# Jackie-Chou/MC-CNN-python

Measured on AMD Instinct MI355X. Metric: Mdisparities/s (HxWxD / s) end-to-end match.py timed region, images resident in HBM, higher is better.
Workload: dtype f32; 1 GPU; cfg2: 750x500 synthetic stereo pair, D=256, one pair per GPU; weights=converted reference checkpoint

## Files before the change

### include/mccnn.h

```cpp
#ifndef MCCNN_H
#define MCCNN_H

#include <stddef.h>
#include <stdint.h>

#ifdef __cplusplus
extern "C" {
#endif

typedef void *mccnn_stream_t;

#define MCCNN_ABI_VERSION 7

#define MCCNN_E_INVALID (-1)
#define MCCNN_E_UNSUPPORTED (-2)
#define MCCNN_E_SCRATCH (-3)

#define MCCNN_SIDE_LEFT 0
#define MCCNN_SIDE_RIGHT 1

int mccnn_version(void);
const char *mccnn_last_error_string(void);

#define MCCNN_CV_EXACT 0
#define MCCNN_CV_MFMA 1
int mccnn_cost_volume(const float *fl, const float *fr, int H, int W, int C, int D, float *lcv, float *rcv, int mode,
                      mccnn_stream_t stream);

int mccnn_cost_volume_hwd(const float *fl, const float *fr, int H, int W, int C, int D, float *lcv_hwd, float *rcv_hwd,
                          int mode, mccnn_stream_t stream);

size_t mccnn_decision_pack_bytes(int n_fc, int units, int mode);
int mccnn_decision_pack(const float *weights, int n_fc, int units, float weight_scale, int mode, void *packed,
                        mccnn_stream_t stream);
int mccnn_cost_volume_accurate(const float *aL, const float *aR, int H, int W, int C, int units, int n_fc, int D,
                               const void *packed, const float *biases, const float *w_final, float b_final,
                               float weight_scale, float *lcv, float *rcv, int mode, int *saturation_flag,
                               mccnn_stream_t stream);
int mccnn_cost_volume_accurate_hwd(const float *aL, const float *aR, int H, int W, int C, int units, int n_fc, int D,
                                   const void *packed, const float *biases, const float *w_final, float b_final,
                                   float weight_scale, float *lcv_hwd, float *rcv_hwd, int mode, int *saturation_flag,
                                   mccnn_stream_t stream);

int mccnn_cost_volume_fill(float *lcv, float *rcv, int D, int H, int W, int pixel_major, mccnn_stream_t stream);

typedef uint32_t mccnn_support_t;
size_t mccnn_support_bytes(int H, int W);
#define MCCNN_SUPPORT_UP(s) ((s) & 31u)
#define MCCNN_SUPPORT_DOWN(s) (((s) >> 5) & 31u)
#define MCCNN_SUPPORT_LEFT(s) (((s) >> 10) & 31u)
#define MCCNN_SUPPORT_RIGHT(s) (((s) >> 15) & 31u)
#define MCCNN_SUPPORT_COUNT(s) ((s) >> 20)
int mccnn_cross_arms(const float *image, int H, int W, float tau, int L, mccnn_support_t *support,
                     mccnn_stream_t stream);
int mccnn_cross_arms_pair(const float *image_left, const float *image_right, int H, int W, float tau, int L,
                          mccnn_support_t *support_left, mccnn_support_t *support_right, mccnn_stream_t stream);
int mccnn_cross_region_list(const mccnn_support_t *support, int H, int W, int L, int32_t *region,
                            mccnn_stream_t stream);

#define MCCNN_CBCA_SEPARABLE 0
#define MCCNN_CBCA_REFERENCE_ORDER 1
int mccnn_cbca_iter(const float *in, float *out, const mccnn_support_t *support, int D, int H, int W, int L, int order,
                    mccnn_stream_t stream);

int mccnn_cbca_iter_pair(const float *in_left, float *out_left, const mccnn_support_t *support_left,
                         const float *in_right, float *out_right, const mccnn_support_t *support_right, int D, int H,
                         int W, int L, int order, mccnn_stream_t stream);

int mccnn_cbca_iter_both(const float *in, float *out, const mccnn_support_t *support_self,
                         const mccnn_support_t *support_other, int D, int H, int W, int L, int side,
                         mccnn_stream_t stream);

int mccnn_cbca_iter_hwd(const float *in_hwd, float *out_hwd, const mccnn_support_t *support, int D, int H, int W, int L,
                        mccnn_stream_t stream);
int mccnn_cbca_iter_hwd_pair(const float *in_left, float *out_left, const mccnn_support_t *support_left,
                             const float *in_right, float *out_right, const mccnn_support_t *support_right, int D,
                             int H, int W, int L, mccnn_stream_t stream);

int mccnn_cbca_iter_hwd_pair_wta(const float *in_left, float *out_left, const mccnn_support_t *support_left,
                                 const float *in_right, float *out_right, const mccnn_support_t *support_right, int D,
                                 int H, int W, int L, float *disparity_left, float *disparity_right, int store_right,
                                 mccnn_stream_t stream);

// ... 116 lines not shown
```

### mc-cnn-python_amd/csrc/cost_volume.hip

```cpp
#include "common.h"

namespace mccnn {

constexpr int CV_TW = 64;
constexpr int CV_DT = 64;
constexpr int CV_C = 64;
#ifndef CVM_WAVES_PER_SIMD
#define CVM_WAVES_PER_SIMD 6
#endif
constexpr int CV_LD = 68;

template <bool PIXEL_MAJOR>
__global__ __launch_bounds__(256) void cost_volume_exact_kernel(const float *__restrict__ fl,
                                                                const float *__restrict__ fr, int H, int W, int D,
                                                                float *__restrict__ lcv, float *__restrict__ rcv, int Dp)
{
    __shared__ __attribute__((aligned(16))) float sR[(CV_TW + CV_DT - 1) * CV_LD];
    __shared__ __attribute__((aligned(16))) float sL[CV_TW * CV_LD];
    const int w0 = blockIdx.x * CV_TW, h = blockIdx.y, d0 = blockIdx.z * CV_DT;
    if (w0 + CV_TW - 1 < d0) return;
    const int tid = threadIdx.x;
    const size_t rowbase = (size_t)h * W;
    for (int i = tid; i < CV_TW * 16; i += 256) {
        const int px = i >> 4, c4 = i & 15;
// ... 506 lines not shown
    const bool left = blockIdx.y == 0;
    const int d = (int)blockIdx.z * 64 + lane;
    const int dmax = min((int)blockIdx.z * 64 + 63, D - 1);
    if ((int)blockIdx.z * 64 >= D) return;
    float *row = (left ? lcv : rcv) + (size_t)h * W * Dp;
    const __amdgpu_buffer_rsrc_t rs = __builtin_amdgcn_make_buffer_rsrc(row, 0, (int)((size_t)W * Dp * 4), 0x00020000);
    const unsigned pix = (unsigned)Dp * 4u;
    const int c_first = left ? dmax + 2 : max(W - dmax - 3, 0), nsteps = left ? c_first + 1 : W - c_first;
    auto col = [&](int t) { return left ? c_first - t : c_first + t; };
    const int voff = d < Dp ? d * 4 : kDrop;
    const int sto = d < D ? voff : kDrop;
    float x1 = 0.f, x2 = 0.f, x3 = 0.f;
    float buf[PF];
    const int dmin = (int)blockIdx.z * 64;
    const int nA = min(nsteps, left ? c_first - dmin + 1 : (W - dmin) - c_first);
    auto issue = [&](int slot, int t) {
        const int c = col(min(t, nA - 1));
        buf[slot] = __uint_as_float(__builtin_amdgcn_raw_buffer_load_b32(rs, voff, (unsigned)c * pix, 0));
    };
    auto third = [](float s) {
        const float zh = 0.3333333432674407958984375f;
        const float q = s * zh;
        const float r = __builtin_fmaf(-3.0f, q, s);
        const float q2 = __builtin_fmaf(r, zh, q);
        return (__builtin_fabsf(s) < __builtin_inff() && s != 0.f) ? q2 : s;
    };
    auto step = [&](int c, bool stored, float have) {
        float s = 0.f - x1;
        s = s - x2;
        s = s - x3;
        const float val = stored ? have : -third(s);
        if (left) { x3 = x2; x2 = x1; x1 = val; }
        else      { x1 = x2; x2 = x3; x3 = val; }
        __builtin_amdgcn_raw_buffer_store_b32(__float_as_uint(val), rs, stored ? kDrop : sto, (unsigned)c * pix, 0);
    };
    if (nA > 0) {
#pragma unroll
        for (int k = 0; k < PF; ++k) issue(k, k);
        for (int t0 = 0; t0 < nA; t0 += PF) {
#pragma unroll
            for (int k = 0; k < PF; ++k) {
                const int t = t0 + k;
                if (t < nA) {
                    const int c = col(t);
                    step(c, left ? c >= d : c < W - d, buf[k]);
                }
                issue(k, t + PF);
            }
        }
    }
    for (int t = max(nA, 0); t < nsteps; ++t) step(col(t), false, 0.f);
}

int launch_cost_volume_fill(float *lcv, float *rcv, int D, int H, int W, hipStream_t s, const char *what)
{
    if (D > 1)
        hipLaunchKernelGGL(cost_volume_fill_kernel, dim3(cdiv(H, 64), D - 1, 2), dim3(64), 0, s, lcv, rcv, D, H, W);
    return check_launch(what);
}

int launch_cost_volume_fill_hwd(float *lcv_hwd, float *rcv_hwd, int D, int Dp, int H, int W, hipStream_t s, const char *what)
{
    if (D > 1) {
#ifdef CV_FILL_FOUR_PER_LANE
        if (Dp <= 256)
            hipLaunchKernelGGL(cost_volume_fill_hwd_kernel<1>, dim3(H, 2), dim3(64), 0, s, lcv_hwd, rcv_hwd, D, Dp, H, W);
        else
            hipLaunchKernelGGL(cost_volume_fill_hwd_kernel<2>, dim3(H, 2), dim3(64), 0, s, lcv_hwd, rcv_hwd, D, Dp, H, W);
#else
        hipLaunchKernelGGL(cost_volume_fill_hwd_lanes_kernel, dim3(H, 2, cdiv(D, 64)), dim3(64), 0, s, lcv_hwd, rcv_hwd, D, Dp,
                           H, W);
#endif
    }
    return check_launch(what);
}

}

extern "C" int mccnn_cost_volume(const float *fl, const float *fr, int H, int W, int C, int D, float *lcv, float *rcv,
                                 int mode, mccnn_stream_t stream)
{
    using namespace mccnn;
    MCCNN_REQUIRE(fl && fr && lcv && rcv, MCCNN_E_INVALID, "mccnn_cost_volume: null pointer");
    MCCNN_REQUIRE(H > 0 && W > 0 && D > 0, MCCNN_E_INVALID, "mccnn_cost_volume: non-positive size");
    MCCNN_REQUIRE(C == CV_C, MCCNN_E_UNSUPPORTED, "mccnn_cost_volume: C=%d, kernels are built for 64 channels", C);
    MCCNN_REQUIRE(D <= W - 2, MCCNN_E_UNSUPPORTED,
                  "mccnn_cost_volume: D=%d needs W >= D+2 (the reference's border recurrence pf:106 is degenerate "
                  "beyond that), W=%d", D, W);
    hipStream_t s = (hipStream_t)stream;
    const dim3 block(256);
    if (mode == MCCNN_CV_EXACT) {
        const dim3 grid(cdiv(W, CV_TW), H, cdiv(D, CV_DT));
        hipLaunchKernelGGL(cost_volume_exact_kernel<false>, grid, block, 0, s, fl, fr, H, W, D, lcv, rcv, 0);
    } else if (mode == MCCNN_CV_MFMA) {
        const int nwt = cdiv(W, 64), nbands = cdiv(D + 63, 64) + 1;
        const long total = (long)nwt * nbands * H;
        MCCNN_REQUIRE(total <= 0x7fffffffL, MCCNN_E_UNSUPPORTED, "mccnn_cost_volume: %ld tiles exceed the grid", total);
        hipLaunchKernelGGL(cost_volume_mfma_kernel<false>, dim3((unsigned)total), block, 0, s, fl, fr, H, W, D, lcv, rcv, nwt,
                           nbands, (int)total, 0);
    } else {
        MCCNN_REQUIRE(false, MCCNN_E_INVALID, "mccnn_cost_volume: unknown mode %d", mode);
    }
    int rc = check_launch("mccnn_cost_volume");
    if (rc) return rc;
    return launch_cost_volume_fill(lcv, rcv, D, H, W, s, "mccnn_cost_volume(fill)");
}

extern "C" int mccnn_cost_volume_hwd(const float *fl, const float *fr, int H, int W, int C, int D, float *lcv_hwd,
                                     float *rcv_hwd, int mode, mccnn_stream_t stream)
{
    using namespace mccnn;
    MCCNN_REQUIRE(fl && fr && lcv_hwd && rcv_hwd, MCCNN_E_INVALID, "mccnn_cost_volume_hwd: null pointer");
    MCCNN_REQUIRE(H > 0 && W > 0 && D > 0, MCCNN_E_INVALID, "mccnn_cost_volume_hwd: non-positive size");
    MCCNN_REQUIRE(C == CV_C, MCCNN_E_UNSUPPORTED, "mccnn_cost_volume_hwd: C=%d, kernels are built for 64 channels", C);
    MCCNN_REQUIRE(D <= W - 2, MCCNN_E_UNSUPPORTED,
                  "mccnn_cost_volume_hwd: D=%d needs W >= D+2 (the reference's border recurrence pf:106 is degenerate "
                  "beyond that), W=%d", D, W);
    MCCNN_REQUIRE(mode == MCCNN_CV_EXACT || mode == MCCNN_CV_MFMA, MCCNN_E_INVALID, "mccnn_cost_volume_hwd: unknown mode %d",
                  mode);
#ifdef CV_FILL_FOUR_PER_LANE
    constexpr int kMaxD = 512;
#else
    constexpr int kMaxD = 1024;
#endif
    MCCNN_REQUIRE(D <= kMaxD, MCCNN_E_UNSUPPORTED, "mccnn_cost_volume_hwd: D=%d > %d", D, kMaxD);
    const int Dp = mccnn_hwd_pitch(D);
    MCCNN_REQUIRE((size_t)W * Dp * 4 < ((size_t)1 << 31), MCCNN_E_UNSUPPORTED,
                  "mccnn_cost_volume_hwd: a %d x %d row exceeds a buffer descriptor's reach", W, D);
    hipStream_t s = (hipStream_t)stream;
    if (mode == MCCNN_CV_MFMA) {
        const int nwt = cdiv(W, 64), nbands = cdiv(D + 63, 64) + 1;
        const long total = (long)nwt * nbands * H;
        MCCNN_REQUIRE(total <= 0x7fffffffL, MCCNN_E_UNSUPPORTED, "mccnn_cost_volume_hwd: %ld tiles exceed the grid", total);
        hipLaunchKernelGGL(cost_volume_mfma_kernel<true>, dim3((unsigned)total), dim3(256), 0, s, fl, fr, H, W, D, lcv_hwd,
                           rcv_hwd, nwt, nbands, (int)total, Dp);
    } else {
#ifdef CV_HWD_TILE_KERNEL
        const dim3 grid(cdiv(W, CV_TW), H, cdiv(D, CV_DT));
        hipLaunchKernelGGL(cost_volume_exact_kernel<true>, grid, dim3(256), 0, s, fl, fr, H, W, D, lcv_hwd, rcv_hwd, Dp);
#else
        const dim3 grid(cdiv(W, CVP_TW), H, 1);
        hipLaunchKernelGGL(cost_volume_exact_pairs_kernel, grid, dim3(256), 0, s, fl, fr, H, W, D, lcv_hwd, rcv_hwd, Dp);
#endif
    }
    int rc = check_launch("mccnn_cost_volume_hwd");
    if (rc) return rc;
    return launch_cost_volume_fill_hwd(lcv_hwd, rcv_hwd, D, Dp, H, W, s, "mccnn_cost_volume_hwd(fill)");
}

extern "C" int mccnn_cost_volume_fill(float *lcv, float *rcv, int D, int H, int W, int pixel_major, mccnn_stream_t stream)
{
    using namespace mccnn;
    MCCNN_REQUIRE(lcv && rcv, MCCNN_E_INVALID, "mccnn_cost_volume_fill: null pointer");
    MCCNN_REQUIRE(H > 0 && W > 0 && D > 0, MCCNN_E_INVALID, "mccnn_cost_volume_fill: non-positive size");
    MCCNN_REQUIRE(D <= W - 2, MCCNN_E_UNSUPPORTED, "mccnn_cost_volume_fill: D=%d needs W >= D+2, W=%d", D, W);
    if (!pixel_major) return launch_cost_volume_fill(lcv, rcv, D, H, W, (hipStream_t)stream, "mccnn_cost_volume_fill");
    const int Dp = mccnn_hwd_pitch(D);
    MCCNN_REQUIRE(D <= 1024, MCCNN_E_UNSUPPORTED, "mccnn_cost_volume_fill: D=%d > 1024", D);
    MCCNN_REQUIRE((size_t)W * Dp * 4 < ((size_t)1 << 31), MCCNN_E_UNSUPPORTED,
                  "mccnn_cost_volume_fill: a %d x %d row exceeds a buffer descriptor's reach", W, D);
    return launch_cost_volume_fill_hwd(lcv, rcv, D, Dp, H, W, (hipStream_t)stream, "mccnn_cost_volume_fill");
}
```

### mc-cnn-python_amd/src/_hipabi.py

```python
import ctypes
import os

import torch

_HERE = os.path.dirname(os.path.abspath(__file__))
LIB_PATH = os.environ.get("MCCNN_HIP_LIB") or os.path.join(os.path.dirname(_HERE), "lib", "libmccnn_hip.so")

MCCNN_ABI_VERSION = 7
MCCNN_CV_EXACT = 0
MCCNN_CV_MFMA = 1
MCCNN_CBCA_SEPARABLE = 0
MCCNN_CBCA_REFERENCE_ORDER = 1
MCCNN_SIDE_LEFT = 0
MCCNN_SIDE_RIGHT = 1
MCCNN_SGM_ACC_STORE = 0
MCCNN_SGM_ACC_ADD = 1
MCCNN_SGM_ACC_ADD_QUARTER = 2
MCCNN_E_INVALID = -1
MCCNN_E_UNSUPPORTED = -2
MCCNN_E_SCRATCH = -3

_vp = ctypes.c_void_p
_i = ctypes.c_int
_f = ctypes.c_float
_sz = ctypes.c_size_t

SIGNATURES = {
    "mccnn_version": (_i, []),
    "mccnn_last_error_string": (ctypes.c_char_p, []),
    "mccnn_cost_volume": (_i, [_vp, _vp, _i, _i, _i, _i, _vp, _vp, _i, _vp]),
    "mccnn_cost_volume_hwd": (_i, [_vp, _vp, _i, _i, _i, _i, _vp, _vp, _i, _vp]),
    "mccnn_cost_volume_fill": (_i, [_vp, _vp, _i, _i, _i, _i, _vp]),
    "mccnn_decision_pack_bytes": (_sz, [_i, _i, _i]),
    "mccnn_decision_pack": (_i, [_vp, _i, _i, _f, _i, _vp, _vp]),
    "mccnn_cost_volume_accurate": (_i, [_vp, _vp, _i, _i, _i, _i, _i, _i, _vp, _vp, _vp, _f, _f, _vp, _vp, _i, _vp, _vp]),
    "mccnn_cost_volume_accurate_hwd": (_i, [_vp, _vp, _i, _i, _i, _i, _i, _i, _vp, _vp, _vp, _f, _f, _vp, _vp, _i, _vp,
                                            _vp]),
    "mccnn_support_bytes": (_sz, [_i, _i]),
    "mccnn_cross_arms": (_i, [_vp, _i, _i, _f, _i, _vp, _vp]),
    "mccnn_cross_arms_pair": (_i, [_vp, _vp, _i, _i, _f, _i, _vp, _vp, _vp]),
    "mccnn_cross_region_list": (_i, [_vp, _i, _i, _i, _vp, _vp]),
    "mccnn_cbca_iter": (_i, [_vp, _vp, _vp, _i, _i, _i, _i, _i, _vp]),
    "mccnn_cbca_iter_pair": (_i, [_vp, _vp, _vp, _vp, _vp, _vp, _i, _i, _i, _i, _i, _vp]),
    "mccnn_cbca_iter_both": (_i, [_vp, _vp, _vp, _vp, _i, _i, _i, _i, _i, _vp]),
    "mccnn_cbca_iter_hwd": (_i, [_vp, _vp, _vp, _i, _i, _i, _i, _vp]),
    "mccnn_cbca_iter_hwd_pair": (_i, [_vp, _vp, _vp, _vp, _vp, _vp, _i, _i, _i, _i, _vp]),
    "mccnn_cbca_iter_hwd_pair_wta": (_i, [_vp, _vp, _vp, _vp, _vp, _vp, _i, _i, _i, _i, _vp, _vp, _i, _vp]),
    "mccnn_cbca_iter_hwd_long": (_i, [_vp, _vp, _vp, _i, _i, _i, _i, _vp]),
    "mccnn_cbca_iter_hwd_long_pair": (_i, [_vp, _vp, _vp, _vp, _vp, _vp, _i, _i, _i, _i, _vp]),
    "mccnn_cbca_prog_bytes": (_sz, [_i, _i, _i]),
    "mccnn_cbca_prog_build_pair": (_i, [_vp, _vp, _i, _i, _i, _i, _vp, _vp, _vp]),
    "mccnn_cbca_iter_prog_pair": (_i, [_vp, _vp, _vp, _vp, _vp, _vp, _vp, _vp, _i, _i, _i, _i, _vp]),
    "mccnn_cbca_prog_build_skip_pair": (_i, [_vp, _vp, _i, _i, _i, _i, _vp, _vp, _vp]),
    "mccnn_cbca_prog_build_both_pair": (_i, [_vp, _vp, _i, _i, _i, _i, _vp, _vp, _vp]),
    "mccnn_cbca_iter_prog_pair_skip": (_i, [_vp, _vp, _vp, _vp, _vp, _vp, _vp, _vp, _i, _i, _i, _i, _vp]),
    "mccnn_cbca_iter_prog": (_i, [_vp, _vp, _vp, _vp, _i, _i, _i, _i, _vp]),
    "mccnn_cbca_iter_prog_skip": (_i, [_vp, _vp, _vp, _vp, _i, _i, _i, _i, _vp]),
    "mccnn_cbca_iter_prog_refresh": (_i, [_vp, _vp, _vp, _vp, _i, _i, _i, _i, _vp]),
    "mccnn_cbca_iter_prog_pair_refresh": (_i, [_vp, _vp, _vp, _vp, _vp, _vp, _vp, _vp, _i, _i, _i, _i, _vp]),
    "mccnn_cbca_iter_prog_pair_wta": (_i, [_vp, _vp, _vp, _vp, _vp, _vp, _vp, _vp, _i, _i, _i, _i, _vp, _vp, _i, _vp]),
    "mccnn_wta_hwd": (_i, [_vp, _i, _i, _i, _vp, _vp]),
    "mccnn_subpixel_hwd": (_i, [_vp, _vp, _i, _i, _i, _i, _vp, _vp]),
    "mccnn_hwd_pitch": (_i, [_i]),
    "mccnn_dhw_to_hwd": (_i, [_vp, _vp, _i, _i, _i, _vp]),
    "mccnn_hwd_to_dhw": (_i, [_vp, _vp, _i, _i, _i, _vp]),
    "mccnn_sgm_scratch_bytes": (_sz, [_i, _i, _i]),
    "mccnn_sgm_pass": (_i, [_vp, _vp, ctypes.POINTER(_vp), ctypes.POINTER(_i), _i, _i, _i, _i, _i, _i,
                            _f, _f, _f, _f, _f, _vp, _sz, _vp]),
    "mccnn_sgm_flags": (_i, [_vp, _vp, _i, _i, _i, _i, _i, _f, _vp, _sz, _vp]),
    "mccnn_sgm_pass_flagged": (_i, [ctypes.POINTER(_vp), ctypes.POINTER(_i), _i, _i, _i, _i, _i, _i, _f, _f, _f, _f, _vp, _sz,
                                    _vp]),
    "mccnn_sgm_pass_accumulate": (_i, [ctypes.POINTER(_vp), ctypes.POINTER(_vp), ctypes.POINTER(_i), _i, _i, _i, _i, _i, _i,
                                       _f, _f, _f, _f, _i, _vp, _sz, _vp]),
    "mccnn_sgm_first_pass": (_i, [_vp, _vp, ctypes.POINTER(_vp), ctypes.POINTER(_vp), ctypes.POINTER(_i), _i, _i, _i,
                                  _i, _f, _f, _f, _f, _f, _vp, _sz, _vp]),
    "mccnn_wta": (_i, [_vp, _i, _i, _i, _vp, _vp]),
    "mccnn_lr_status": (_i, [_vp, _vp, _i, _i, _i, _vp, _vp]),
    "mccnn_interpolate": (_i, [_vp, _vp, _i, _i, _vp, _vp]),
    "mccnn_interpolate_ex": (_i, [_vp, _vp, _i, _i, _i, _i, _vp, _vp]),
    "mccnn_subpixel": (_i, [_vp, _vp, _i, _i, _i, _vp, _vp]),
    "mccnn_subpixel_ex": (_i, [_vp, _vp, _i, _i, _i, _i, _vp, _vp]),
    "mccnn_median": (_i, [_vp, _i, _i, _i, _i, _vp, _vp]),
    "mccnn_bilateral": (_i, [_vp, _vp, _i, _i, _i, _i, _vp, _f, _vp, _vp]),
    "mccnn_bias_act": (_i, [_vp, _vp, _i, _i, ctypes.c_long, _i, _vp]),
# ... 64 lines not shown
```

### mc-cnn-python_amd/src/stereo_device.py

```python
import ctypes
import math

import numpy as np
import torch

import _hipabi as hip


def _f32(x):
    return float(np.float32(x))


class StageTimer(object):

    def __init__(self, enabled=False):
        self.enabled = enabled
        self.records = []
        self.spans = []
        self._open = None

    def start(self, name):
        if not self.enabled:
            return
        ev = torch.cuda.Event(enable_timing=True)
# ... 79 lines not shown
    lib = hip.load()
    packed = torch.empty((lib.mccnn_conv3x3_split_weights_bytes(),), dtype=torch.uint8, device=w.device)
    hip.check(lib.mccnn_conv3x3_split_pack(hip.ptr(w), scale, hip.ptr(packed), hip.stream()), "mccnn_conv3x3_split_pack")
    return packed, scale


def conv1_split(images, weight, bias, pad, act_scale=SPLIT_ACT_SCALE, sat_flag=None):
    N, H, W = images.shape
    assert tuple(weight.shape) == (64, 1, 3, 3) and images.is_contiguous() and weight.is_contiguous()
    out = torch.empty((N, H + 2 * pad - 2, W + 2 * pad - 2, 256), dtype=torch.uint8, device=images.device)
    hip.check(hip.load().mccnn_conv1_split(hip.ptr(images), hip.ptr(weight), hip.ptr(bias), hip.ptr(out), N, H, W,
                                           int(pad), float(act_scale), hip.ptr(sat_flag) if sat_flag is not None else None,
                                           hip.stream()), "mccnn_conv1_split")
    return out


def conv3x3_split(x, packed, weight_scale, bias, last, act_scale=SPLIT_ACT_SCALE, sat_flag=None):
    N, Hi, Wi, rec = x.shape
    assert rec == 256 and x.dtype == torch.uint8 and x.is_contiguous()
    if last:
        out = torch.empty((N, Hi - 2, Wi - 2, 64), dtype=torch.float32, device=x.device)
    else:
        out = torch.empty((N, Hi - 2, Wi - 2, 256), dtype=torch.uint8, device=x.device)
    hip.check(hip.load().mccnn_conv3x3_split(hip.ptr(x), hip.ptr(packed), hip.ptr(bias), hip.ptr(out), N, Hi, Wi,
                                             float(weight_scale), float(act_scale), 1 if last else 0,
                                             hip.ptr(sat_flag) if sat_flag is not None else None, hip.stream()),
              "mccnn_conv3x3_split")
    return out


def cost_volume(fl, fr, ndisp, mode=hip.MCCNN_CV_EXACT, out=None):
    H, W, C = fl.shape
    if out is None:
        lcv = torch.empty((ndisp, H, W), dtype=torch.float32, device=fl.device)
        rcv = torch.empty((ndisp, H, W), dtype=torch.float32, device=fl.device)
    else:
        lcv, rcv = out
    hip.check(hip.load().mccnn_cost_volume(hip.ptr(fl), hip.ptr(fr), H, W, C, int(ndisp), hip.ptr(lcv), hip.ptr(rcv),
                                           int(mode), hip.stream()), "mccnn_cost_volume")
    return lcv, rcv


def cost_volume_hwd(fl, fr, ndisp, out=None, mode=hip.MCCNN_CV_EXACT):
    H, W, C = fl.shape
    dp = hwd_pitch(ndisp)
    if out is None:
        lcv = torch.zeros((H, W, dp), dtype=torch.float32, device=fl.device)
        rcv = torch.zeros((H, W, dp), dtype=torch.float32, device=fl.device)
    else:
        lcv, rcv = out
    hip.check(hip.load().mccnn_cost_volume_hwd(hip.ptr(fl), hip.ptr(fr), H, W, C, int(ndisp), hip.ptr(lcv), hip.ptr(rcv),
                                               int(mode), hip.stream()), "mccnn_cost_volume_hwd")
    return lcv, rcv


DECISION_UNITS = 384
DECISION_MAPS = (64, 112)
DECISION_FC_LAYERS = (3, 4)
DECISION_MAX_D = 1024
DECISION_LIBRARY_BYTES = 256 << 20


def decision_kernel_refusal(net, W, D):
    if net.num_conv_feature_maps not in DECISION_MAPS:
        return "%d feature maps (the decision kernel serves %s)" % (net.num_conv_feature_maps, " or ".join(
            str(c) for c in DECISION_MAPS))
    if net.num_fc_units != DECISION_UNITS:
        return "%d units per hidden layer (the decision kernel is built for %d)" % (net.num_fc_units, DECISION_UNITS)
    if net.num_fc_layers not in DECISION_FC_LAYERS:
        return "%d fully-connected layers (the decision kernel serves 3 or 4)" % net.num_fc_layers
    if D < 2 or D > DECISION_MAX_D:
        return "ndisp=%d outside [2, %d]" % (D, DECISION_MAX_D)
    if D > W - 2:
        return "ndisp=%d needs an image at least ndisp + 2 pixels wide (W=%d)" % (D, W)
    return None


def decision_pack(weights, n_fc, mode):
    lib = hip.load()
    w = weights.detach().contiguous().float()
    units = int(w.shape[-1])
    nbytes = int(lib.mccnn_decision_pack_bytes(int(n_fc), units, int(mode)))
    if nbytes == 0 or tuple(w.shape) != (n_fc - 1, units, units):
        raise hip.MccnnHipError("mccnn_decision_pack: %d fc layers of %d units are outside the decision kernel's "
                                "envelope (3 or 4 layers of %d units)" % (n_fc, units, DECISION_UNITS))
    m = float(w.abs().max())
    scale = 2.0 ** math.floor(math.log2(1024.0 / m)) if m > 0.0 and math.isfinite(m) else 1.0
    packed = torch.empty((nbytes,), dtype=torch.uint8, device=w.device)
    hip.check(lib.mccnn_decision_pack(hip.ptr(w), int(n_fc), units, scale, int(mode), hip.ptr(packed), hip.stream()),
              "mccnn_decision_pack")
    return packed, scale


def cost_volume_fill(lcv, rcv, ndisp, pixel_major):
    H, W = (lcv.shape[0], lcv.shape[1]) if pixel_major else (lcv.shape[1], lcv.shape[2])
    hip.check(hip.load().mccnn_cost_volume_fill(hip.ptr(lcv), hip.ptr(rcv), int(ndisp), H, W, 1 if pixel_major else 0,
                                                hip.stream()), "mccnn_cost_volume_fill")
    return lcv, rcv


def accurate_scores_library(net, aL, aR, ndisp, lcv, rcv, pixel_major, budget=DECISION_LIBRARY_BYTES):
    H, W, U = aL.shape
    ws = [w.detach() for w in net.fc_weights]
    bs = [b.detach() for b in net.fc_biases]
    lv = lcv.permute(2, 0, 1) if pixel_major else lcv
    rv = rcv.permute(2, 0, 1) if pixel_major else rcv
# ... 634 lines not shown


DEFAULT_HP = dict(cbca_intensity=0.02, cbca_distance=14, cbca_num_iterations1=2, cbca_num_iterations2=16,
                  sgm_P1=2.3, sgm_P2=55.9, sgm_Q1=4, sgm_Q2=8, sgm_D=0.08, sgm_V=1.5, blur_sigma=6,
                  blur_threshold=2)


SGM_MAX_D = 1024
COST_VOLUME_HWD_MAX_D = 1024
DECISION_AUTO = "kernel"


def check_envelope(H, W, D):
    H, W, D = int(H), int(W), int(D)
    if H < 1 or W < 1:
        raise ValueError("%dx%d: empty image" % (W, H))
    if D < 2 or D > SGM_MAX_D:
        raise ValueError("ndisp=%d outside [2, %d]: SGM is built for at most %d disparities" % (D, SGM_MAX_D, SGM_MAX_D))
    if D > W - 2:
        raise ValueError("ndisp=%d needs an image at least ndisp + 2 = %d pixels wide, got W=%d" % (D, D + 2, W))


def workspace_bytes(H, W, D, pixel_major=True, cbca_kernel="auto", pairs_in_flight=1, arch="fast",
                    fc_units=DECISION_UNITS):
    check_envelope(H, W, D)
    lib = hip.load()
    H, W, D = int(H), int(W), int(D)
    dp = (D + 3) & ~3
    n = 4 * H * W * dp * 4
    n += 5 * int(lib.mccnn_sgm_scratch_bytes(H, W, D))
    n += 2 * int(lib.mccnn_support_bytes(H, W))
    n += H * W * 4 + 6 * H * W * 4
    if pixel_major and cbca_kernel != "hwd":
        n += 2 * int(lib.mccnn_cbca_prog_bytes(D, H, W))
    if arch not in ("fast", "accurate"):
        raise ValueError("arch must be 'fast' or 'accurate'")
    if arch == "accurate":
        n += 2 * H * W * int(fc_units) * 4
    return n * max(1, int(pairs_in_flight))


def _require_device_memory(nbytes, what):
    free, _total = torch.cuda.mem_get_info()
    avail = free + torch.cuda.memory_reserved() - torch.cuda.memory_allocated()
    if nbytes > avail:
        raise RuntimeError("%s needs %.2f GB of device memory, %.2f GB are available" % (what, nbytes / 1e9, avail / 1e9))


class StereoMatcher(object):

    def __init__(self, net, hp=None, cv_mode=hip.MCCNN_CV_EXACT, cbca_order=hip.MCCNN_CBCA_REFERENCE_ORDER,
                 feature_tile_rows=None, extras=None, features="auto", layout="auto", cbca_kernel="auto",
                 on_saturation="fallback", skip_unit_regions=True, two_chains=True, free_chains=True, refresh_first=True,
                 sgm_flags_once=True, decision="auto"):
        self.device = hip.require_device()
        self.net = net
        self.hp = dict(DEFAULT_HP)
        if hp:
            self.hp.update(hp)
        self.cv_mode = cv_mode
        self.cbca_order = cbca_order
        self.feature_tile_rows = feature_tile_rows
        if features not in ("auto", "miopen", "split_f16"):
            raise ValueError("features must be 'auto', 'miopen' or 'split_f16'")
        if features == "split_f16" and feature_tile_rows is not None:
            raise ValueError("row banding is implemented for the library convolutions only")
        if features == "auto":
            features = "split_f16" if (feature_tile_rows is None and net.supports_split_features()) else "miopen"
        self.features = features
        if decision not in ("auto", "kernel", "library"):
            raise ValueError("decision must be 'auto', 'kernel' or 'library'")
        self.accurate = hasattr(net, "fc_weights")
        self.decision = decision
        if self.accurate and features == "split_f16":
            raise ValueError("the split-operand feature kernels are built for the fast network")
        if layout not in ("auto", "plane_major"):
            raise ValueError("layout must be 'auto' or 'plane_major'")
        self.layout = layout
        if cbca_kernel not in ("auto", "prog", "hwd"):
            raise ValueError("cbca_kernel must be 'auto', 'prog' or 'hwd'")
        self.cbca_kernel = cbca_kernel
        if on_saturation not in ("fallback", "raise", "ignore"):
            raise ValueError("on_saturation must be 'fallback', 'raise' or 'ignore'")
        self.on_saturation = on_saturation
        self._library_twin = None
        self._decision_ran = None
        self.skip_unit_regions = bool(skip_unit_regions)
        self.two_chains = bool(two_chains)
        self.free_chains = bool(free_chains)
        self.refresh_first = bool(refresh_first)
        self.sgm_flags_once = bool(sgm_flags_once)
        self.extras = dict(both_view_support=False, interpolation_directions=4, occlusion_from_left=False,
                           numpy1_promotion=False, sgm_independent_directions=False)
        if extras:
            unknown = set(extras) - set(self.extras)
            if unknown:
                raise ValueError("unknown extras: %s" % sorted(unknown))
            self.extras.update(extras)
        self._ws = {}
        self._graphs = {}
        self._side = None
        self._right = None
        self._ingest = None

    def _right_stream(self):
        if self._right is None:
            self._right = torch.cuda.Stream()
        return self._right

    def features_saturated(self, reset=True):
        return self.net.split_saturated(reset)

    def saturation_checked(self):
        return self.features == "split_f16" or (self.accurate and self._decision_ran == "kernel")

    def saturation_notice(self):
        if self.accurate:
            return "activations left the matrix-core decision kernel's range: {} repeated on the float32 library decision route"
        return ("activations left the matrix-core feature kernels' range: {} repeated with the float32 library "
                "convolutions")

    def workspace(self, H, W, D):
        key = (H, W, D)
        ws = self._ws.get(key)
        if ws is None:
            need = workspace_bytes(H, W, D, self.pixel_major(), self.workspace_cbca_kernel(H, W, D),
                                   arch="accurate" if self.accurate else "fast",
                                   fc_units=self.net.num_fc_units if self.accurate else DECISION_UNITS)
            self._ws, self._graphs = {}, {}
            _require_device_memory(need, "StereoMatcher: the workspace of a %dx%d pair with ndisp=%d" % (W, H, D))
            dp = hwd_pitch(D)
            n = H * W * dp
            dev = self.device
            ws = dict(
                vol=[torch.empty((n,), dtype=torch.float32, device=dev) for _ in range(4)],
                scratch=sgm_scratch(H, W, D, dev),
                sgm_flags=[sgm_scratch(H, W, D, dev) for _ in SGM_DIRECTIONS],
                sup_l=support_buffer(H, W, dev), sup_r=support_buffer(H, W, dev),
                status=torch.empty((H, W), dtype=torch.int32, device=dev),
                maps=torch.empty((6, H, W), dtype=torch.float32, device=dev),
            )
            if self.accurate:
                ws["halves"] = tuple(torch.empty((H, W, self.net.num_fc_units), dtype=torch.float32, device=dev)
                                     for _ in range(2))
# ... 42 lines not shown
            if redo is not None:
                return redo
        return res

    def _side_work(self, ws, L, R, D, want_flags):
        hp = self.hp
        if self._side is None:
            self._side = torch.cuda.Stream()
        self._side.wait_stream(torch.cuda.current_stream())
        with torch.cuda.stream(self._side):
            sup_l, sup_r = cross_arms_pair(L, R, hp["cbca_intensity"], hp["cbca_distance"], ws["sup_l"], ws["sup_r"])
            if ws["progs"] is not None:
                cbca_prog_build_pair(sup_l, sup_r, D, hp["cbca_distance"], ws["progs"],
                                     "both" if self.skip_unit_regions else "full")
            flag_planes = sgm_flag_planes(L, R, D, hp["sgm_D"], out=ws["sgm_flags"]) if want_flags else None
            ready = torch.cuda.Event()
            ready.record(self._side)
        return sup_l, sup_r, flag_planes, ready

    def _side_work_timed(self, ws, L, R, D, timer):
        hp = self.hp
        timer.start("cross_arms")
        sup_l, sup_r = cross_arms_pair(L, R, hp["cbca_intensity"], hp["cbca_distance"], ws["sup_l"], ws["sup_r"])
        timer.stop()
        if ws["progs"] is not None:
            timer.start("cbca_prog_build")
            cbca_prog_build_pair(sup_l, sup_r, D, hp["cbca_distance"], ws["progs"])
            timer.stop()
        return sup_l, sup_r

    def decision_route(self, W, D):
        if self.decision == "library":
            return "library"
        why = decision_kernel_refusal(self.net, W, D)
        if why is None:
            return DECISION_AUTO if self.decision == "auto" else "kernel"
        if self.decision == "kernel":
            raise ValueError("decision='kernel': %s" % why)
        import warnings
        warnings.warn("accurate network: %s; the decision stage runs on the float32 library route" % why)
        return "library"

    def _cost_volumes_accurate(self, ws, fl, fr, D, dhw, hwd, timer):
        direct = self.pixel_major() and D <= COST_VOLUME_HWD_MAX_D
        route = self.decision_route(fl.shape[1], D)
        self._decision_ran = route
        timer.start("cost_volume")
        left, right = cost_volume_accurate(self.net, fl, fr, D, mode=self.cv_mode, decision=route, pixel_major=direct,
                                           out=(hwd[2], hwd[3]) if direct else (dhw[0], dhw[1]), halves=ws["halves"],
                                           sat_flag=self.net._split_flag() if route == "kernel" else None)
        timer.stop()
        return left, right, direct

    def _cost_volumes(self, fl, fr, D, dhw, hwd, timer, ws=None):
        if self.accurate:
            return self._cost_volumes_accurate(ws, fl, fr, D, dhw, hwd, timer)
        direct = self.pixel_major() and D <= COST_VOLUME_HWD_MAX_D
        timer.start("cost_volume")
        if direct:
            left, right = cost_volume_hwd(fl, fr, D, out=(hwd[2], hwd[3]), mode=self.cv_mode)
        else:
            left, right = cost_volume(fl, fr, D, self.cv_mode, out=(dhw[0], dhw[1]))
        timer.stop()
        return left, right, direct

    def _sgm_hp(self):
        return [self.hp[k] for k in ("sgm_P1", "sgm_P2", "sgm_Q1", "sgm_Q2", "sgm_D", "sgm_V")]

    def _wta_hwd(self, lh, rh, D, m, timer):
        timer.start("wta")
        dl, dr = wta_hwd(lh, D, out=m[0]), wta_hwd(rh, D, out=m[1])
        timer.stop()
        return dl, dr

    def _pixel_major_free(self, ws, L, R, D, left, right, sups, flag_planes, fuse, m, timer):
        hp, progs, dist = self.hp, ws["progs"], self.hp["cbca_distance"]
        n1, n2 = int(hp["cbca_num_iterations1"]), int(hp["cbca_num_iterations2"])
        if flag_planes is None and self.sgm_flags_once:
            timer.start("sgm_flags")
            flag_planes = sgm_flag_planes(L, R, D, hp["sgm_D"], out=ws["sgm_flags"])
            timer.stop()
        if flag_planes is None and "scratch2" not in ws:
            ws["scratch2"] = sgm_scratch(L.shape[0], L.shape[1], D, self.device)
        chain = dict(skip_unit_regions=self.skip_unit_regions, refresh_first=self.refresh_first, timer=timer)
        main_s, right_s = torch.cuda.current_stream(), self._right_stream()
        right_s.wait_stream(main_s)
        ends = []
        for st, (v, t), sup, prog, side, scr in ((main_s, left, sups[0], progs[0], hip.MCCNN_SIDE_LEFT, ws["scratch"]),
                                                 (right_s, right, sups[1], progs[1], hip.MCCNN_SIDE_RIGHT, ws.get("scratch2"))):
            with torch.cuda.stream(st):
                timer.span_start("aggregation_1")
                v, t = cbca_prog_chain(v, t, sup, prog, D, n1, dist, **chain)
                timer.span_stop("aggregation_1")
                timer.span_start("sgm")
                if self.extras["sgm_independent_directions"]:
                    (v,), (t,) = sgm_average_independent_hwd(L, R, [v], [t], [side], D, *self._sgm_hp(), scr, timer,
                                                             flags=flag_planes)
                else:
                    sgm_average_hwd(L, R, [v], [side], D, *self._sgm_hp(), scr, timer, flags=flag_planes)
                timer.span_stop("sgm")
                timer.span_start("aggregation_2")
                v, t = cbca_prog_chain(v, t, sup, prog, D, n2 - 1 if fuse else n2, dist, total=n2, fused_last=fuse, **chain)
                timer.span_stop("aggregation_2")
                ends.append((v, t))
        main_s.wait_stream(right_s)
        (lh, lt), (rh, rt) = ends
        if not fuse:
            return self._wta_hwd(lh, rh, D, m, timer) + (lh,)
        _prog_launch_wta((lh, lt, sups[0], progs[0]), (rh, rt, sups[1], progs[1]), D, dist, (m[0], m[1]), False, timer)
        return m[0], m[1], lt
# ... 71 lines not shown
            timer.stop()
        if keep is not None:
            keep["sgm"] = (lcv.clone(), rcv.clone())
        (lcv, t1d), (rcv, t2d) = self._aggregate_dhw((lcv, t1d), (rcv, t2d), sups, hp["cbca_num_iterations2"], timer)
        if keep is not None:
            keep["cbca2"] = (lcv.clone(), rcv.clone())
        timer.start("wta")
        dl, dr = wta(lcv, out=m[0]), wta(rcv, out=m[1])
        timer.stop()
        return dl, dr, lcv

    def _post(self, ws, L, D, dl, dr, left_volume, pixel_major, m, timer, keep, out, static_out):
        hp, ex = self.hp, self.extras
        if out is not None and (tuple(out.shape) != tuple(L.shape) or out.dtype != torch.float32 or not out.is_contiguous()
                                or out.device != L.device):
            raise ValueError("match: `out` must be a contiguous float32 [H,W] tensor on the images' device")
        timer.start("post")
        st = lr_status(dl, dr, D, out=ws["status"] if keep is None else None)
        di = interpolate(dl, st, out=m[2], directions=ex["interpolation_directions"],
                         occlusion_from_left=ex["occlusion_from_left"])
        if pixel_major:
            ds = subpixel_hwd(di, left_volume, D, out=m[3], numpy1_promotion=ex["numpy1_promotion"])
        else:
            ds = subpixel(di, left_volume, out=m[3], numpy1_promotion=ex["numpy1_promotion"])
        dm = median(ds, 5, 5, out=m[4])
        db = bilateral(L, dm, 5, 5, 0, hp["blur_sigma"], hp["blur_threshold"], out=out if out is not None else m[5])
        timer.stop()
        if keep is not None:
            keep.update(wta=(dl, dr), status=st, interp=di, subpixel=ds, median=dm, bilateral=db)
            return db
        return db if (static_out or out is not None) else db.clone()

    def _match(self, left_image, right_image, ndisp, timer=_NO_TIMER, keep=None, _static_out=False, out=None):
        L = left_image.reshape(left_image.shape[0], left_image.shape[1]).contiguous()
        R = right_image.reshape(right_image.shape[0], right_image.shape[1]).contiguous()
        H, W = L.shape
        D = int(ndisp)
        ws = self.workspace(H, W, D)
        dp = hwd_pitch(D)
        dhw = [b[:D * H * W].view(D, H, W) for b in ws["vol"]]
        hwd = [b[:H * W * dp].view(H, W, dp) for b in ws["vol"]]
        overlap = timer is _NO_TIMER
        free = self.free_chains and self.two_chains and keep is None and ws["progs"] is not None
        flag_planes = None

        timer.start("features")
        if self.features == "split_f16":
            fl, fr = self.net.features_pair_hwc_split(L, R)
        else:
            fl, fr = self.net.features_pair_hwc(L, R, tile_rows=self.feature_tile_rows)
        timer.stop()
        if overlap:
            sup_l, sup_r, flag_planes, ready = self._side_work(ws, L, R, D, want_flags=free and self.sgm_flags_once)
        lv, rv, pixel_major = self._cost_volumes(fl, fr, D, dhw, hwd, timer, ws)
        del fl, fr
        if keep is not None:
            keep["cv"] = (hwd_to_dhw(lv, D), hwd_to_dhw(rv, D)) if pixel_major else (lv.clone(), rv.clone())
        if overlap:
            torch.cuda.current_stream().wait_event(ready)
        else:
            sup_l, sup_r = self._side_work_timed(ws, L, R, D, timer)
        sups = (sup_l, sup_r)

        m = ws["maps"] if keep is None else torch.empty_like(ws["maps"])
        if self.pixel_major():
            if not pixel_major:
                timer.start("cv_to_pixel_major")
                lv, rv = dhw_to_hwd(lv, hwd[2]), dhw_to_hwd(rv, hwd[3])
                timer.stop()
            fuse = (int(self.hp["cbca_num_iterations2"]) >= 1 and D <= cbca_hwd_wta_max_d()
                    and int(self.hp["cbca_distance"]) <= CBCA_HWD_MAX_DISTANCE)
            if free:
                dl, dr, left_volume = self._pixel_major_free(ws, L, R, D, (lv, hwd[0]), (rv, hwd[1]), sups, flag_planes,
                                                             fuse, m, timer)
            else:
                dl, dr, left_volume = self._pixel_major_joined(ws, L, R, D, (lv, hwd[0]), (rv, hwd[1]), sups, fuse, m,
                                                               timer, keep)
        else:
            dl, dr, left_volume = self._plane_major(ws, L, R, D, (lv, dhw[2]), (rv, dhw[3]), hwd, sups, m, timer, keep)
        return self._post(ws, L, D, dl, dr, left_volume, self.pixel_major(), m, timer, keep, out, _static_out)

    def _ingest_buffers(self, H, W):
        b = self._ingest
        if b is None or b[0] != (H, W):
            dev = self.device
            b = ((H, W), torch.empty((H, W), dtype=torch.float32, device=dev),
                 torch.empty((H, W), dtype=torch.float32, device=dev), ingest_scratch(H, W, dev))
            self._ingest = b
        return b[1:]

    def match_u8(self, left_u8, right_u8, ndisp, out=None):
        H, W, _ = _u8_image(left_u8)
        sl, sr, scratch = self._ingest_buffers(H, W)
        left_u8 = left_u8.to(self.device, non_blocking=True).contiguous()
        right_u8 = right_u8.to(self.device, non_blocking=True).contiguous()
        ingest_u8_pair(left_u8, right_u8, sl, sr, scratch)
        return self.match(sl, sr, ndisp, out=out)

    def _capture(self, key, shape, make_static, prologue=None):
        H, W, D = shape
        self.workspace(H, W, D)
        self._side = self._right = None
        static = make_static()
        side = torch.cuda.Stream()
        side.wait_stream(torch.cuda.current_stream())
        with torch.cuda.stream(side):
            for _ in range(2):
# ... 56 lines not shown
```

Measured before the change: 11460 Mdisparities/s.

## Split cost volume into scores and border kernels on concurrent streams

```diff
diff --git a/include/mccnn.h b/include/mccnn.h
--- a/include/mccnn.h
+++ b/include/mccnn.h
@@ -29,6 +29,11 @@
 
 int mccnn_cost_volume_hwd(const float *fl, const float *fr, int H, int W, int C, int D, float *lcv_hwd, float *rcv_hwd,
                           int mode, mccnn_stream_t stream);
+
+int mccnn_cost_volume_hwd_scores(const float *fl, const float *fr, int H, int W, int C, int D, float *lcv_hwd,
+                                 float *rcv_hwd, mccnn_stream_t stream);
+int mccnn_cost_volume_hwd_border(const float *fl, const float *fr, int H, int W, int C, int D, float *lcv_hwd,
+                                 float *rcv_hwd, mccnn_stream_t stream);
 
 size_t mccnn_decision_pack_bytes(int n_fc, int units, int mode);
 int mccnn_decision_pack(const float *weights, int n_fc, int units, float weight_scale, int mode, void *packed,
diff --git a/mc-cnn-python_amd/csrc/cost_volume.hip b/mc-cnn-python_amd/csrc/cost_volume.hip
--- a/mc-cnn-python_amd/csrc/cost_volume.hip
+++ b/mc-cnn-python_amd/csrc/cost_volume.hip
@@ -582,6 +582,76 @@
     for (int t = max(nA, 0); t < nsteps; ++t) step(col(t), false, 0.f);
 }
 
+template <bool LEFT>
+__device__ __forceinline__ void cv_border_side(const float *__restrict__ fl, const float *__restrict__ fr,
+                                               float *__restrict__ vol, int D, int Dp, int W, int h, int dblock, int lane)
+{
+    constexpr int kDrop = 0x7ffffff0;
+    const int d = dblock * 64 + lane;
+    const int dmax = min(dblock * 64 + 63, D - 1);
+    float *row = vol + (size_t)h * W * Dp;
+    const __amdgpu_buffer_rsrc_t rs = __builtin_amdgcn_make_buffer_rsrc(row, 0, (int)((size_t)W * Dp * 4), 0x00020000);
+    const unsigned pix = (unsigned)Dp * 4u;
+    const int sto = d < D ? d * 4 : kDrop;
+    const int c0 = LEFT ? d : W - d - 3;
+    const size_t rowbase = (size_t)h * W;
+    auto seed = [&](int k) {
+        const int lp = LEFT ? min(d + k, W - 1) : W - 3 + k, rp = LEFT ? k : max(W - d - 3 + k, 0);
+        const float4 *a = reinterpret_cast<const float4 *>(fl + (rowbase + lp) * CV_C);
+        const float4 *b = reinterpret_cast<const float4 *>(fr + (rowbase + rp) * CV_C);
+        float acc[8];
+#pragma unroll
+        for (int i = 0; i < 8; ++i) {
+            const float4 a0 = a[2 * i], a1 = a[2 * i + 1], b0 = b[2 * i], b1 = b[2 * i + 1];
+            const float p[8] = {a0.x * b0.x, a0.y * b0.y, a0.z * b0.z, a0.w * b0.w,
+                                a1.x * b1.x, a1.y * b1.y, a1.z * b1.z, a1.w * b1.w};
+#pragma unroll
+            for (int j = 0; j < 8; ++j) acc[j] = i == 0 ? p[j] : acc[j] + p[j];
+        }
+        float s = ((acc[0] + acc[1]) + (acc[2] + acc[3])) + ((acc[4] + acc[5]) + (acc[6] + acc[7]));
+        s = 0.f + s;
+        return -1.f * s;
+    };
+    const float seed0 = seed(0), seed1 = seed(1), seed2 = seed(2);
+    float x1 = 0.f, x2 = 0.f, x3 = 0.f;
+    auto third = [](float s) {
+        const float zh = 0.3333333432674407958984375f;
+        const float q = s * zh;
+        const float r = __builtin_fmaf(-3.0f, q, s);
+        const float q2 = __builtin_fmaf(r, zh, q);
+        return (__builtin_fabsf(s) < __builtin_inff() && s != 0.f) ? q2 : s;
+    };
+    auto step = [&](int c, bool stored, float have) {
+        float s = 0.f - x1;
+        s = s - x2;
+        s = s - x3;
+        const float val = stored ? have : -third(s);
+        if (LEFT) { x3 = x2; x2 = x1; x1 = val; }
+        else      { x1 = x2; x2 = x3; x3 = val; }
+        __builtin_amdgcn_raw_buffer_store_b32(__float_as_uint(val), rs, stored ? kDrop : sto, (unsigned)c * pix, 0);
+    };
+    const int cend = LEFT ? -1 : W, dc = LEFT ? -1 : 1;
+    for (int c = LEFT ? dmax + 2 : W - dmax - 3; c != cend; c += dc) {
+        const int k = c - c0;
+        float have = seed2;
+        have = k == 1 ? seed1 : have;
+        have = k == 0 ? seed0 : have;
+        step(c, LEFT ? c >= d : c < W - d, have);
+    }
+}
+
+__global__ __launch_bounds__(64) void cost_volume_border_hwd_kernel(const float *__restrict__ fl,
+                                                                    const float *__restrict__ fr,
+                                                                    float *__restrict__ lcv, float *__restrict__ rcv,
+                                                                    int D, int Dp, int H, int W)
+{
+    if ((int)blockIdx.z * 64 >= D) return;
+    if (blockIdx.y == 0)
+        cv_border_side<true>(fl, fr, lcv, D, Dp, W, blockIdx.x, blockIdx.z, threadIdx.x);
+    else
+        cv_border_side<false>(fl, fr, rcv, D, Dp, W, blockIdx.x, blockIdx.z, threadIdx.x);
+}
+
 int launch_cost_volume_fill(float *lcv, float *rcv, int D, int H, int W, hipStream_t s, const char *what)
 {
     if (D > 1)
@@ -603,6 +673,30 @@
 #endif
     }
     return check_launch(what);
+}
+
+int launch_cost_volume_border_hwd(const float *fl, const float *fr, float *lcv_hwd, float *rcv_hwd, int D, int Dp, int H,
+                                  int W, hipStream_t s, const char *what)
+{
+    if (D > 1)
+        hipLaunchKernelGGL(cost_volume_border_hwd_kernel, dim3(H, 2, cdiv(D, 64)), dim3(64), 0, s, fl, fr, lcv_hwd, rcv_hwd,
+                           D, Dp, H, W);
+    return check_launch(what);
+}
+
+int check_cost_volume_hwd_args(const char *name, const void *fl, const void *fr, int H, int W, int C, int D,
+                               const void *lcv_hwd, const void *rcv_hwd)
+{
+    MCCNN_REQUIRE(fl && fr && lcv_hwd && rcv_hwd, MCCNN_E_INVALID, "%s: null pointer", name);
+    MCCNN_REQUIRE(H > 0 && W > 0 && D > 0, MCCNN_E_INVALID, "%s: non-positive size", name);
+    MCCNN_REQUIRE(C == CV_C, MCCNN_E_UNSUPPORTED, "%s: C=%d, kernels are built for 64 channels", name, C);
+    MCCNN_REQUIRE(D <= W - 2, MCCNN_E_UNSUPPORTED,
+                  "%s: D=%d needs W >= D+2 (the reference's border recurrence pf:106 is degenerate beyond that), W=%d",
+                  name, D, W);
+    MCCNN_REQUIRE(D <= 1024, MCCNN_E_UNSUPPORTED, "%s: D=%d > 1024", name, D);
+    MCCNN_REQUIRE((size_t)W * mccnn_hwd_pitch(D) * 4 < ((size_t)1 << 31), MCCNN_E_UNSUPPORTED,
+                  "%s: a %d x %d row exceeds a buffer descriptor's reach", name, W, D);
+    return 0;
 }
 
 }
@@ -678,6 +772,27 @@
     return launch_cost_volume_fill_hwd(lcv_hwd, rcv_hwd, D, Dp, H, W, s, "mccnn_cost_volume_hwd(fill)");
 }
 
+extern "C" int mccnn_cost_volume_hwd_scores(const float *fl, const float *fr, int H, int W, int C, int D, float *lcv_hwd,
+                                            float *rcv_hwd, mccnn_stream_t stream)
+{
+    using namespace mccnn;
+    const int rc = check_cost_volume_hwd_args("mccnn_cost_volume_hwd_scores", fl, fr, H, W, C, D, lcv_hwd, rcv_hwd);
+    if (rc) return rc;
+    hipLaunchKernelGGL(cost_volume_exact_pairs_kernel, dim3(cdiv(W, CVP_TW), H, 1), dim3(256), 0, (hipStream_t)stream, fl,
+                       fr, H, W, D, lcv_hwd, rcv_hwd, mccnn_hwd_pitch(D));
+    return check_launch("mccnn_cost_volume_hwd_scores");
+}
+
+extern "C" int mccnn_cost_volume_hwd_border(const float *fl, const float *fr, int H, int W, int C, int D, float *lcv_hwd,
+                                            float *rcv_hwd, mccnn_stream_t stream)
+{
+    using namespace mccnn;
+    const int rc = check_cost_volume_hwd_args("mccnn_cost_volume_hwd_border", fl, fr, H, W, C, D, lcv_hwd, rcv_hwd);
+    if (rc) return rc;
+    return launch_cost_volume_border_hwd(fl, fr, lcv_hwd, rcv_hwd, D, mccnn_hwd_pitch(D), H, W, (hipStream_t)stream,
+                                         "mccnn_cost_volume_hwd_border");
+}
+
 extern "C" int mccnn_cost_volume_fill(float *lcv, float *rcv, int D, int H, int W, int pixel_major, mccnn_stream_t stream)
 {
     using namespace mccnn;
diff --git a/mc-cnn-python_amd/src/_hipabi.py b/mc-cnn-python_amd/src/_hipabi.py
--- a/mc-cnn-python_amd/src/_hipabi.py
+++ b/mc-cnn-python_amd/src/_hipabi.py
@@ -30,6 +30,8 @@
     "mccnn_last_error_string": (ctypes.c_char_p, []),
     "mccnn_cost_volume": (_i, [_vp, _vp, _i, _i, _i, _i, _vp, _vp, _i, _vp]),
     "mccnn_cost_volume_hwd": (_i, [_vp, _vp, _i, _i, _i, _i, _vp, _vp, _i, _vp]),
+    "mccnn_cost_volume_hwd_scores": (_i, [_vp, _vp, _i, _i, _i, _i, _vp, _vp, _vp]),
+    "mccnn_cost_volume_hwd_border": (_i, [_vp, _vp, _i, _i, _i, _i, _vp, _vp, _vp]),
     "mccnn_cost_volume_fill": (_i, [_vp, _vp, _i, _i, _i, _i, _vp]),
     "mccnn_decision_pack_bytes": (_sz, [_i, _i, _i]),
     "mccnn_decision_pack": (_i, [_vp, _i, _i, _f, _i, _vp, _vp]),
diff --git a/mc-cnn-python_amd/src/stereo_device.py b/mc-cnn-python_amd/src/stereo_device.py
--- a/mc-cnn-python_amd/src/stereo_device.py
+++ b/mc-cnn-python_amd/src/stereo_device.py
@@ -155,6 +155,26 @@
     hip.check(hip.load().mccnn_cost_volume_hwd(hip.ptr(fl), hip.ptr(fr), H, W, C, int(ndisp), hip.ptr(lcv), hip.ptr(rcv),
                                                int(mode), hip.stream()), "mccnn_cost_volume_hwd")
     return lcv, rcv
+
+
+def _cost_volume_hwd_part(entry, fl, fr, ndisp, out):
+    H, W, C = fl.shape
+    dp = hwd_pitch(ndisp)
+    if out is None:
+        out = (torch.zeros((H, W, dp), dtype=torch.float32, device=fl.device),
+               torch.zeros((H, W, dp), dtype=torch.float32, device=fl.device))
+    lcv, rcv = out
+    hip.check(getattr(hip.load(), entry)(hip.ptr(fl), hip.ptr(fr), H, W, C, int(ndisp), hip.ptr(lcv), hip.ptr(rcv),
+                                         hip.stream()), entry)
+    return lcv, rcv
+
+
+def cost_volume_hwd_scores(fl, fr, ndisp, out=None):
+    return _cost_volume_hwd_part("mccnn_cost_volume_hwd_scores", fl, fr, ndisp, out)
+
+
+def cost_volume_hwd_border(fl, fr, ndisp, out=None):
+    return _cost_volume_hwd_part("mccnn_cost_volume_hwd_border", fl, fr, ndisp, out)
 
 
 DECISION_UNITS = 384
@@ -895,7 +915,7 @@
     def __init__(self, net, hp=None, cv_mode=hip.MCCNN_CV_EXACT, cbca_order=hip.MCCNN_CBCA_REFERENCE_ORDER,
                  feature_tile_rows=None, extras=None, features="auto", layout="auto", cbca_kernel="auto",
                  on_saturation="fallback", skip_unit_regions=True, two_chains=True, free_chains=True, refresh_first=True,
-                 sgm_flags_once=True, decision="auto"):
+                 sgm_flags_once=True, decision="auto", cost_volume_schedule="split"):
         self.device = hip.require_device()
         self.net = net
         self.hp = dict(DEFAULT_HP)
@@ -933,6 +953,9 @@
         self.free_chains = bool(free_chains)
         self.refresh_first = bool(refresh_first)
         self.sgm_flags_once = bool(sgm_flags_once)
+        if cost_volume_schedule not in ("split", "serial"):
+            raise ValueError("cost_volume_schedule must be 'split' or 'serial'")
+        self.cost_volume_schedule = cost_volume_schedule
         self.extras = dict(both_view_support=False, interpolation_directions=4, occlusion_from_left=False,
                            numpy1_promotion=False, sgm_independent_directions=False)
         if extras:
@@ -1081,10 +1104,18 @@
         timer.stop()
         return left, right, direct
 
-    def _cost_volumes(self, fl, fr, D, dhw, hwd, timer, ws=None):
+    def _cost_volumes(self, fl, fr, D, dhw, hwd, timer, ws=None, split=False):
         if self.accurate:
             return self._cost_volumes_accurate(ws, fl, fr, D, dhw, hwd, timer)
         direct = self.pixel_major() and D <= COST_VOLUME_HWD_MAX_D
+        if split and direct and self.cv_mode == hip.MCCNN_CV_EXACT:
+            main_s, right_s = torch.cuda.current_stream(), self._right_stream()
+            right_s.wait_stream(main_s)
+            with torch.cuda.stream(right_s):
+                cost_volume_hwd_border(fl, fr, D, out=(hwd[2], hwd[3]))
+            left, right = cost_volume_hwd_scores(fl, fr, D, out=(hwd[2], hwd[3]))
+            main_s.wait_stream(right_s)
+            return left, right, direct
         timer.start("cost_volume")
         if direct:
             left, right = cost_volume_hwd(fl, fr, D, out=(hwd[2], hwd[3]), mode=self.cv_mode)
@@ -1262,7 +1293,8 @@
         timer.stop()
         if overlap:
             sup_l, sup_r, flag_planes, ready = self._side_work(ws, L, R, D, want_flags=free and self.sgm_flags_once)
-        lv, rv, pixel_major = self._cost_volumes(fl, fr, D, dhw, hwd, timer, ws)
+        lv, rv, pixel_major = self._cost_volumes(fl, fr, D, dhw, hwd, timer, ws,
+                                                 split=overlap and free and self.cost_volume_schedule == "split")
         del fl, fr
         if keep is not None:
             keep["cv"] = (hwd_to_dhw(lv, D), hwd_to_dhw(rv, D)) if pixel_major else (lv.clone(), rv.clone())
```

Result: no change. 11520 Mdisparities/s, median of 4 (+0.5%).
